# yizhiwang96/Slice3D

Hardware: AMD Instinct MI355X
Metric: occupancy query-points/sec (U-Net encode + per-query decode, 256^2 x 12 slices) (higher is better)
Workload: dtype f16x3

## Files before the change

slice3d_amd/csrc/api.hip:

```cpp
#include <dlfcn.h>
#include <stdarg.h>
#include <string.h>

#include <vector>
#include <mutex>

#include <math.h>

#include "conv_plan.h"
#include "decode.h"
#include "train.h"
#include "ldm_ops.h"

static thread_local char g_err[512] = "";

void s3d_set_error(const char* fmt, ...) {
    va_list ap;
    va_start(ap, fmt);
    vsnprintf(g_err, sizeof(g_err), fmt, ap);
    va_end(ap);
}

extern "C" int s3d_version(void) { return S3D_VERSION; }
extern "C" const char* s3d_last_error(void) { return g_err; }
// ... 85 lines not shown
        tot += ms;
    }
    *total_ms = tot;
    *count = (long)g_prof_ev[id].size();
    return 0;
}

#define TRY(x)              \
    do {                    \
        int rc__ = (x);     \
        if (rc__) return rc__; \
    } while (0)

static const int kEncCin[13] = {3, 64, 64, 128, 128, 256, 256, 256, 512, 512, 512, 512, 512};
static const int kEncCout[13] = {64, 64, 128, 128, 256, 256, 256, 512, 512, 512, 512, 512, 512};
static const bool kEncTap[13] = {false, true, false, true, false, false, true,
                                 false, false, true, false, false, true};
static const int kUpC[4] = {512, 256, 128, 64};

struct PackedConv {
    size_t w, scale, shift;
    size_t w16;
    int cout_pad, KU;
};
struct EncLayout {
    PackedConv enc[13];
    size_t pool_scale[4], pool_shift[4];
};
struct UNetLayout {
    EncLayout E;
    PackedConv trans_up[4], up_t[4], up_c1[4], up_c2[4], outc;
    PackedConv trans_cx, trans_ce;
// ... 182 lines not shown
    }
    TRY(pack_linear(P->outc.w, base + L.outc.w, 3, 16, 32, 32, 0, st));
    TRY(pack_linear(P->outc.w, base + L.outc.w16, 3, 16, 32, 32, 0, st, 1));
    TRY(launch_fold_bn(P->outc.b, nullptr, base + L.outc.scale, base + L.outc.shift, 3, 16, 1, 0, st));
    hipError_t e = hipMemcpyAsync(base + L.emds, P->emds, (size_t)P->n_slices * 128 * sizeof(float),
                                  hipMemcpyDeviceToDevice, st);
    if (e != hipSuccess) {
        s3d_set_error("unet_pack: memcpy failed: %s", hipGetErrorString(e));
        return (int)e;
    }
    return pack_unet_slice_terms(base, L, P->n_slices, st);
}

#define S3D_SPLITK_FLOATS ((size_t)4718592)
struct UNetWs {
    size_t in16, a, b, x[5], p[4], proj, pre, mid, splitk;
    size_t lat, up1_u, up1_pre;
    size_t total;
};
static UNetWs unet_ws(int B, int S, int ns) {
    UNetWs W;
    size_t off = 0;
    auto take = [&](size_t n) {
        size_t o = off;
        off += (n + 63) / 64 * 64;
        return o;
    };
    const size_t px = (size_t)B * S * S;
    W.in16 = take(px * 16);
    W.a = take(px * 64);
    W.b = take(px * 64 / 2);
    const int xc[5] = {64, 128, 256, 512, 512};
    for (int i = 0; i < 5; ++i) W.x[i] = take((px >> (2 * i)) * xc[i]);
    for (int i = 0; i < 4; ++i) W.p[i] = take((px >> (2 * (i + 1))) * xc[i]);
    W.proj = take(px * 32);
    W.pre = take(px * 32);
    W.mid = take(px * ns * 32);
    W.splitk = take(S3D_SPLITK_FLOATS);
    W.lat = take(px / 256 * 512);
    W.up1_u = take(px / 64 * 256);
    W.up1_pre = take(px / 64 * 256);
    W.total = off;
    return W;
}

extern "C" size_t s3d_unet_workspace_bytes(int batch, int size, int n_slices) {
    return unet_ws(batch, size, n_slices).total * sizeof(float);
}

static ConvLaunch conv_desc(const float* base, const PackedConv& pc, int prec, int N, int H, int W, int ks, int act) {
    ConvLaunch c = {};
// ... 38 lines not shown
        c.out_mode = S3D_OUT_CONVT;
        c.cout_store = 256;
        TRY(launch_conv(c, st));
    }
    {
        ConvLaunch c = conv_desc(base, L.up_c1[0], S3D_PREC_F32, ns, 4, 4, 3, S3D_ACT_NONE);
        c.scale = c.shift = nullptr;
        c.nsrc = 1;
        c.src[0] = plain_src(base + L.up1_tab_in, 256);
        c.out = base + L.up1_tab;
        TRY(launch_conv(c, st));
    }
    return 0;
}

static int encoder_fwd(const float* base, const EncLayout& E, int prec, int N, int S, int first, const float* in,
                       float* const tap[5], float* const pp[2], float* const pool[4], float* splitk, hipStream_t st) {
    const float* cur = in;
    int curC = first ? kEncCout[0] : 16, res = S, tap_i = 0, flip = first;
    for (int i = first; i < 13; ++i) {
        ConvLaunch c = conv_desc(base, E.enc[i], prec, N, res, res, 3, kEncTap[i] ? S3D_ACT_NONE : S3D_ACT_RELU);
        c.nsrc = 1;
        c.src[0] = plain_src(cur, curC);
        c.splitk_ws = splitk; c.splitk_floats = S3D_SPLITK_FLOATS;
        c.out = kEncTap[i] ? tap[tap_i] : pp[flip];
        TRY(launch_conv(c, st));
        cur = c.out;
        curC = kEncCout[i];
        if (!kEncTap[i]) {
            flip ^= 1;
            continue;
        }
        if (tap_i < 4) {
            TRY(launch_bn_relu_pool(tap[tap_i], base + E.pool_scale[tap_i], base + E.pool_shift[tap_i], pool[tap_i], N,
                                    res, res, curC, st));
            cur = pool[tap_i];
            res /= 2;
        }
        ++tap_i;
    }
    return 0;
}

extern "C" int s3d_unet_encode_fwd(const void* packed, const float* img, const S3dPyramid* out,
                                   float* slices_rec, int B, int S, int ns, int prec, void* workspace,
                                   size_t workspace_bytes, void* stream) {
    hipStream_t st = (hipStream_t)stream;
    S3D_CHECK_ARG(prec == S3D_PREC_F32 || prec == S3D_PREC_F16X3 || prec == S3D_PREC_F16 || prec == S3D_PREC_BF16,
                  "unet_encode: precision mode %d", prec);
    if (prec == S3D_PREC_BF16) prec = S3D_PREC_F16;
    S3D_CHECK_ARG(packed && img && out && workspace, "unet_encode: null argument");
    S3D_CHECK_ARG(B >= 1 && S >= 16 && S % 16 == 0, "unet_encode: B=%d S=%d (S must be a multiple of 16)", B, S);
    S3D_CHECK_ARG(ns >= 1 && ns <= 12, "unet_encode: n_slices %d", ns);
    S3D_CHECK_ARG(out->n_img == B * ns && out->size == S, "unet_encode: pyramid handle mismatch");
    const UNetLayout L = unet_layout(ns);
    const UNetWs W = unet_ws(B, S, ns);
    if (workspace_bytes < W.total * sizeof(float)) {
        s3d_set_error("unet_encode: workspace %zu < %zu bytes", workspace_bytes, W.total * sizeof(float));
        return S3D_E_WORKSPACE;
    }
    const float* base = (const float*)packed;
    float* ws = (float*)workspace;

    ProfScope prof_(S3D_PROF_UNET, st);
    float* const pp[2] = {ws + W.a, ws + W.b};
    float* const tap[5] = {ws + W.x[0], ws + W.x[1], ws + W.x[2], ws + W.x[3], ws + W.x[4]};
    float* const pool[4] = {ws + W.p[0], ws + W.p[1], ws + W.p[2], ws + W.p[3]};
    TRY(launch_conv3x3_first(img, 3, base + L.enc0_raw, nullptr, pp[0], B, S, S, st, base + L.E.enc[0].scale,
                             base + L.E.enc[0].shift, 1));
    TRY(encoder_fwd(base, L.E, prec, B, S, 1, pp[0], tap, pp, pool, ws + W.splitk, st));
    const int r5 = S / 16;
    {
        ConvLaunch c = conv_desc(base, L.trans_cx, prec, B, r5, r5, 1, S3D_ACT_NONE);
        c.scale = c.shift = nullptr;
        c.nsrc = 1;
        c.src[0] = plain_src(ws + W.x[4], 512);
        c.out = ws + W.lat;
        TRY(launch_conv(c, st));
    }
    TRY(launch_slice_bcast_add(ws + W.lat, base + L.slice_v, out->level[0], B, ns, (long)r5 * r5, 512, st));
    const float* prev = out->level[0];
    int rp = r5;
    for (int i = 0; i < 4; ++i) {
        const int C = kUpC[i], Ct = C / 2, ro = rp * 2;
        {
            ConvLaunch c = conv_desc(base, L.trans_up[i], prec, B, ro, ro, 1, S3D_ACT_NONE);
            c.nsrc = 1;
            c.src[0] = plain_src(ws + W.x[3 - i], C);
            c.out = ws + W.proj;
            TRY(launch_conv(c, st));
        }
        {
            ConvLaunch c = conv_desc(base, L.up_c1s[i], prec, B, ro, ro, 3, S3D_ACT_NONE);
            c.scale = c.shift = nullptr;
            c.nsrc = 1;
            c.src[0] = plain_src(ws + W.proj, Ct);
            c.out = ws + W.pre;
            TRY(launch_conv(c, st));
        }
        if (i == 0) {
            {
                ConvLaunch c = conv_desc(base, L.up_t[0], prec, B, rp, rp, 1, S3D_ACT_NONE);
                c.scale = c.shift = nullptr;
                c.nsrc = 1;
                c.src[0] = plain_src(ws + W.lat, C);
                c.out = ws + W.up1_u;
                c.out_mode = S3D_OUT_CONVT;
                c.cout_store = Ct;
                TRY(launch_conv(c, st));
            }
            {
                ConvLaunch c = conv_desc(base, L.up_c1[0], prec, B, ro, ro, 3, S3D_ACT_NONE);
                c.scale = c.shift = nullptr;
                c.nsrc = 1;
                c.src[0] = plain_src(ws + W.up1_u, Ct);
                c.pre = ws + W.pre; c.pre_bdiv = 1;
                c.out = ws + W.up1_pre;
                TRY(launch_conv(c, st));
            }
            TRY(launch_slice_table_act(ws + W.up1_pre, base + L.up1_tab, base + L.up_c1[0].scale, base + L.up_c1[0].shift,
                                       ws + W.mid, B, ns, ro, Ct, st));
        } else {
            ConvLaunch c = {};
            c.wpk16 = prec != S3D_PREC_F32 ? (const void*)(base + L.up_cc[i].w16) : nullptr;
            c.single_pass = prec == S3D_PREC_F16;
            c.N = B * ns; c.H = rp; c.W = rp; c.ks = 2; c.up2x = 1;
            c.CoutPad = Ct; c.wpk = base + L.up_cc[i].w; c.KU = L.up_cc[i].KU;
            c.scale = base + L.up_c1[i].scale; c.shift = base + L.up_c1[i].shift;
            c.act = S3D_ACT_RELU; c.out_mode = S3D_OUT_NHWC; c.cout_store = Ct; c.out_cstride = Ct;
            c.nsrc = 1;
            c.src[0] = plain_src(prev, C);
            c.pre = ws + W.pre; c.pre_bdiv = ns;
            c.pre_tab = base + L.up_tb[i];
            c.out = ws + W.mid;
            TRY(launch_conv(c, st));
        }
        {
            ConvLaunch c = conv_desc(base, L.up_c2[i], prec, B * ns, ro, ro, 3, S3D_ACT_RELU);
            c.nsrc = 1;
            c.src[0] = plain_src(ws + W.mid, Ct);
            c.out = out->level[i + 1];
            TRY(launch_conv(c, st));
        }
        prev = out->level[i + 1];
        rp = ro;
    }
    if (slices_rec) {
        ConvLaunch c = conv_desc(base, L.outc, prec, B * ns, S, S, 1, S3D_ACT_TANH);
        c.nsrc = 1;
        c.src[0] = plain_src(prev, 32);
        c.out = slices_rec;
        c.out_mode = S3D_OUT_NCHW;
        c.cout_store = 3;
        TRY(launch_conv(c, st));
    }
    return 0;
}

static const int kVggCin[14] = {3, 64, 64, 128, 128, 256, 256, 256, 256, 512, 512, 512, 512, 512};
static const int kVggCout[14] = {64, 64, 128, 128, 256, 256, 256, 256, 512, 512, 512, 512, 512, 512};
static const int kVggPoolAfter[14] = {0, 1, 0, 1, 0, 0, 0, 1, 0, 0, 0, 1, 0, 0};
static const int kVggTap[14] = {0, 1, 0, 2, 0, 3, 0, 0, 0, 4, 0, 0, 0, 5};
static const float kVggW[5] = {1.0f / 2.6f, 1.0f / 4.8f, 1.0f / 3.7f, 1.0f / 5.6f, 10.0f / 1.5f};

struct VggLayout {
    PackedConv conv[14];
    size_t mean, stdv, total;
};
static VggLayout vgg_layout() {
    VggLayout L;
    size_t off = 0;
// ... 279 lines not shown
    return false;
}

extern "C" size_t s3d_decode_workspace_bytes(int batch, long n_qry, int n_slices) {
    return decode_ws(batch, n_qry, n_slices, S3D_CHUNK_GROUPS).total * sizeof(float);
}
extern "C" size_t s3d_decode_workspace_bytes_min(int batch, long n_qry, int n_slices) {
    return decode_ws(batch, n_qry, n_slices, S3D_CHUNK_GROUPS_MIN).total * sizeof(float);
}

struct DecodeLanes {
    std::mutex mu;
    hipStream_t aux = nullptr;
    hipEvent_t stagger = nullptr, join = nullptr;
    bool ok = false;
};
static std::atomic<int> g_decode_lanes{-1};
extern "C" int s3d_decode_set_lanes(int n) {
    S3D_CHECK_ARG(n == 1 || n == 2, "decode_set_lanes: %d (1 or 2)", n);
    g_decode_lanes.store(n, std::memory_order_relaxed);
    return 0;
}
static int decode_lanes() {
    int v = g_decode_lanes.load(std::memory_order_relaxed);
    if (v < 0) {
        const char* e = getenv("S3D_DECODE_LANES");
        v = (e && atoi(e) == 2) ? 2 : 1;
        g_decode_lanes.store(v, std::memory_order_relaxed);
    }
    return v;
// ... 8 lines not shown
    if (L.ok) return true;
    hipStream_t s = nullptr;
    hipEvent_t e0 = nullptr, e1 = nullptr;
    const bool made = hipStreamCreateWithFlags(&s, hipStreamNonBlocking) == hipSuccess &&
                      hipEventCreateWithFlags(&e0, hipEventDisableTiming) == hipSuccess &&
                      hipEventCreateWithFlags(&e1, hipEventDisableTiming) == hipSuccess;
    if (!made) {
        if (e1) (void)hipEventDestroy(e1);
        if (e0) (void)hipEventDestroy(e0);
        if (s) (void)hipStreamDestroy(s);
        (void)hipGetLastError();
        return false;
    }
    L.aux = s; L.stagger = e0; L.join = e1; L.ok = true;
    return true;
}
#define S3D_LANES_MIN_GROUPS 8192

static LayerPtrs layer_ptrs(const float* b, const HeadLayout& H, int l) {
    LayerPtrs p;
    p.inw = b + H.L[l].inw; p.inb = b + H.L[l].inb; p.outw = b + H.L[l].outw; p.outb = b + H.L[l].outb;
    p.ln1g = b + H.L[l].ln1g; p.ln1b = b + H.L[l].ln1b; p.w1 = b + H.L[l].w1; p.b1 = b + H.L[l].b1;
    p.w2 = b + H.L[l].w2; p.b2 = b + H.L[l].b2; p.ln2g = b + H.L[l].ln2g; p.ln2b = b + H.L[l].ln2b;
    p.wf16 = b + H.L[l].wf16;
    p.aq16 = b + H.L[l].aq16;
    p.wfb16 = b + H.L[l].wfb16;
    p.aqb16 = b + H.L[l].aqb16;
    return p;
}

// ... 309 lines not shown

extern "C" int s3d_nchw_to_nhwc(const float* in, float* out, int n, int c, int h, int w, void* stream) {
    S3D_CHECK_ARG(in && out, "nchw_to_nhwc: null argument");
    return launch_nchw_to_nhwc(in, out, n, c, h, w, c, (hipStream_t)stream);
}

extern "C" int s3d_nhwc_to_nchw(const float* in, float* out, int n, int c, int h, int w, void* stream) {
    S3D_CHECK_ARG(in && out, "nhwc_to_nchw: null argument");
    return launch_nhwc_to_nchw(in, out, n, c, h, w, (hipStream_t)stream);
}

#include "api_gt.inc"
#include "api_ldm.inc"
#include "api_ldm_ae.inc"
#include "api_train.inc"
#include "api_train_gt.inc"
```

slice3d_amd/csrc/conv.h:

```cpp
#pragma once
#include "common.h"
#include "dropout.h"

struct ConvSrc {
    const float* p;
    int C;
    int bdiv, bmod, sbcast;
};

#define S3D_GN_SLICES 64
#define S3D_GN_CMAX 1536
struct ConvGn {
    const float* table;
    int silu;
};

enum { S3D_ACT_NONE = 0, S3D_ACT_RELU = 1, S3D_ACT_TANH = 2 };
enum { S3D_OUT_NHWC = 0, S3D_OUT_CONVT = 1, S3D_OUT_NCHW = 2 };

struct ConvLaunch {
    ConvSrc src[2];
    int nsrc;
    int N, H, W;
    int ks;
// ... 17 lines not shown
    int xcd_remap;
    const float* gate;
    float gate_scale;
    unsigned long long drop_base;
    float* splitk_ws;
    size_t splitk_floats;
    DropCfg drop;
    ConvGn gn;
    const float* pre;
    int pre_bdiv, pre_bmod;
    int* splits_out;
    int up2x;
    const float* pre_tab;
    int tap_oy, tap_ox;
    int out_py, out_px;
};

int launch_conv(const ConvLaunch& a, hipStream_t stream);
int launch_conv_splitk_finish(const ConvLaunch& a, int nsplit, hipStream_t stream);

enum { S3D_PACK_LINEAR = 0, S3D_PACK_CONV = 1, S3D_PACK_CONVT = 2, S3D_PACK_CONV_DGRAD = 3,
       S3D_PACK_CONVT_DGRAD = 4, S3D_PACK_LINEAR_T = 5 };
struct PackArgs {
    const float* src;
    float* dst;
    int kind;
    int n_valid, n_pad;
    int KU_total, u_off, ku_seg;
    int ld, k_valid;
    int taps, cseg, cseg_valid, cin_tot, cin_begin;
// ... 45 lines not shown
```

slice3d_amd/csrc/conv.hip:

```cpp
#include <stdlib.h>
#include "conv_plan.h"
#include <utility>
#include <vector>

template <int MT, int NT>
__device__ __forceinline__ void conv_epilogue(const ConvLaunch& a, f32x4 (&acc)[MT][NT], const int (&pn)[MT],
                                              const int (&py)[MT], const int (&px)[MT], const bool (&pv)[MT],
                                              int jt0, int g) {
    const bool convt32 = a.out_mode == S3D_OUT_CONVT && a.cout_store % 32 == 0;
    if (NT % 2 == 0 && (a.out_mode == S3D_OUT_NHWC || convt32)) {
        const int m = threadIdx.x & 15;
        const bool lo = m < 8;
#pragma unroll
        for (int np = 0; np < NT / 2; ++np) {
            const int co = (jt0 + 2 * np) * 16 + 16 * (m >> 3) + 4 * g;
            const f32x4 sc = a.scale ? ld4(a.scale + co) : f32x4{1.f, 1.f, 1.f, 1.f};
            const f32x4 sh = a.shift ? ld4(a.shift + co) : zero4();
            const int ct = a.cout_store, cq = convt32 ? co / ct : 0, ccol = convt32 ? co - cq * ct : co;
            const bool col_ok = convt32 ? cq < 4 : co < a.cout_store;
#pragma unroll
            for (int mt = 0; mt < MT; ++mt) {
                f32x4 val[2];
                s3d_full_line_pair(acc[mt][2 * np], acc[mt][2 * np + 1], m, val[0], val[1]);
                const long ob = convt32 ? ((long)(pn[mt] * 2 * a.H + 2 * py[mt] + (cq >> 1)) * (2 * a.W) + 2 * px[mt] + (cq & 1)) * ct
// ... 1067 lines not shown
            const f32x4 v0 = ld4(src + (size_t)k * stride), v1 = ld4(src + (size_t)(k + 1) * stride),
                        v2 = ld4(src + (size_t)(k + 2) * stride), v3 = ld4(src + (size_t)(k + 3) * stride);
            __builtin_amdgcn_sched_barrier(0);
            s += (v0 + v1) + (v2 + v3);
        }
        for (; k < nsplit; ++k) s += ld4(src + (size_t)k * stride);
        f32x4 acc[1][1] = {{s}};
        const int n = (int)(p / ((long)a.H * a.W));
        const int r = (int)(p - (long)n * a.H * a.W);
        const int pn[1] = {n}, py[1] = {r / a.W}, px[1] = {r % a.W};
        const bool pv[1] = {true};
        conv_epilogue<1, 1>(a, acc, pn, py, px, pv, co >> 4, (co >> 2) & 3);
    }
}

int launch_conv_splitk_finish(const ConvLaunch& a, int nsplit, hipStream_t stream) {
    hipLaunchKernelGGL(conv_splitk_finish_kernel, dim3(conv_splitk_finish_blocks(a)), dim3(256), 0, stream, a, nsplit);
    S3D_LAUNCH_CHECK();
    return 0;
}


#define C3S_HP 160
#define C3S_HP1 64
__device__ __forceinline__ int c3s_div(int q, int magic) { return (q * magic) >> 16; }
template <int PT, bool GN, int TAPS = 9>
__global__ __launch_bounds__(256) void conv3x3_small_f16x3_kernel(const ConvLaunch a, int chunks_per_split) {
    constexpr int BORD = TAPS == 9 ? 1 : 0;
    __shared__ __attribute__((aligned(16))) _Float16 s_in[2][2][C3S_HP * C3_PXS];
    const int lane = threadIdx.x & 63, wave = threadIdx.x >> 6;
    const int m = lane & 15, g = lane >> 4;
// ... 194 lines not shown
        if (e.family == p.family && std::equal(e.targ, e.targ + 7, p.targ)) {
            k = &e;
            break;
        }
    S3D_CHECK_ARG(k, "conv: the plan names a kernel instantiation that is not built");
    for (int par = 0; par < (p.per_parity ? 4 : 1); ++par) {
        if (p.per_parity) {
            a.wpk = a_in.wpk + (size_t)par * (a.CoutPad / 16) * a.KU * 256;
            a.out_py = par >> 1; a.out_px = par & 1;
            a.tap_oy = a.out_py - 1; a.tap_ox = a.out_px - 1;
        }
        k->launch(a, p, stream);
        S3D_LAUNCH_CHECK();
    }
    if (a.splits_out) *a.splits_out = p.splits;
    return p.finish ? launch_conv_splitk_finish(a, p.splits, stream) : 0;
}
#undef CK_ARGS
#undef CK
#undef CK_TILE
#undef CK_LDS
#undef CK_SMALL
#undef CK_UP2X
#undef CK_STREAM

__device__ __forceinline__ void pack_frag_body(const PackArgs& a) {
    const long total = (long)(a.n_pad / 16) * a.ku_seg * 256;
    for (long idx = (long)blockIdx.x * blockDim.x + threadIdx.x; idx < total;
         idx += (long)gridDim.x * blockDim.x) {
        int e, lane, ul, j, k;
        if (!a.f16) {
// ... 490 lines not shown
```

slice3d_amd/csrc/conv_plan.h:

```cpp
#pragma once
#include <stdlib.h>
#include <algorithm>
#include "conv.h"

struct ConvTuning {
    bool small3_on, small1_on;
    long small3_pmax, small1_pmax;
};
inline ConvTuning conv_tuning_from_env() {
    const char *e3 = getenv("S3D_CONV_SMALL"), *e1 = getenv("S3D_CONV_SMALL_1X1");
    const int v3 = e3 ? atoi(e3) : 1, v1 = e1 ? atoi(e1) : 1;
    return {v3 != 0, v1 != 0, v3 > 1 ? v3 : 32, v1 > 1 ? v1 : 64};
}
const ConvTuning& conv_tuning();

enum ConvFamily { CONV_IGEMM, CONV_IGEMM_F16X3, CONV_LIN_ROWS, CONV_LIN_STREAM, CONV_LDS, CONV_SMALL, CONV_UP2X_LDS, CONV_N_FAMILIES };
static const struct { const char* name; int nargs; const char* bools; } kConvFamily[CONV_N_FAMILIES] = {
    {"conv_igemm_kernel", 7, "0000011"},       {"conv_igemm_f16x3_kernel", 6, "000001"}, {"lin_rows_f16x3_kernel", 0, ""},
    {"lin_stream_f16x3_kernel", 1, "0"},       {"conv3x3_lds_f16x3_kernel", 6, "000011"}, {"conv3x3_small_f16x3_kernel", 3, "010"},
    {"conv_up2x_lds_f16x3_kernel", 7, "0000000"}};

struct ConvPlan {
    int err;
    ConvFamily family;
    int targ[7];
    unsigned grid_x, grid_y, block;
    int splits, chunks_per_split;
    int tiles_x, tiles_y;
    long n_tasks;
    bool finish;
    bool per_parity;
};

constexpr long kSmallHalo = 160, kSmallHalo1 = 64;
constexpr int kLinRowsTile = 192;

inline bool conv_same_grid(const ConvLaunch& a) { return !((a.Hin && a.Hin != a.H) || (a.Win && a.Win != a.W)); }
inline bool conv_chunked_sources(const ConvLaunch& a) {
    for (int s = 0; s < a.nsrc; ++s)
        if (a.src[s].C % 32 || a.src[s].sbcast) return false;
    return true;
}
inline bool conv_splittable(const ConvLaunch& a) { return a.splitk_ws && a.out_mode == S3D_OUT_NHWC; }
inline bool conv_below_lds_tile(int H, int W) { return W < 16 || H < 8; }
inline int conv_splitk_finish_blocks(const ConvLaunch& a) {
    const long total = (long)(((size_t)a.N * a.H * a.W * a.CoutPad) >> 2);
    return (int)((total + 255) / 256 < 2048 ? (total + 255) / 256 : 2048);
}

inline void conv_plan_splits(ConvPlan& p, const ConvLaunch& a, long nblk_k, bool may_split) {
    int nchunk = 0;
    for (int s = 0; s < a.nsrc; ++s) nchunk += a.src[s].C >> 5;
    const size_t out_floats = (size_t)a.N * a.H * a.W * a.CoutPad;
    int splits = 1;
    long best = -1;
    for (int sp = 1; may_split && sp <= nchunk && (size_t)sp * out_floats <= a.splitk_floats; ++sp) {
        const int c = (nchunk + sp - 1) / sp, se = (nchunk + c - 1) / c;
        if (se != sp) continue;
        const long rounds = (nblk_k * se + 511) / 512;
        const long cost = rounds * (2 * c + 3) + (se > 1 ? 1 + se / 8 : 0);
        if (best < 0 || cost < best) {
// ... 17 lines not shown

inline int conv_plan_route(const ConvLaunch& a, const ConvTuning& t, ConvPlan& p) {
    S3D_CHECK_ARG(a.ks >= 1 && a.ks <= 3, "conv: ks must be 1, 2 or 3");
    S3D_CHECK_ARG(!a.pad_origin || (a.ks == 3 && a.stride > 1 && a.out_mode == S3D_OUT_NHWC),
                  "conv: pad_origin is served for strided 3x3 convolutions only");
    S3D_CHECK_ARG(a.CoutPad % 16 == 0 && a.CoutPad > 0, "conv: CoutPad %d", a.CoutPad);
    for (int s = 0; s < a.nsrc; ++s)
        S3D_CHECK_ARG(a.src[s].C % 16 == 0 && a.src[s].bdiv >= 1, "conv: bad source %d", s);
    S3D_CHECK_ARG(a.out_mode != S3D_OUT_CONVT || (a.drop.p <= 0.f && !a.gate && !a.residual && !a.out_accumulate),
                  "conv: ConvTranspose output takes no dropout / gate / residual / accumulate");
    S3D_CHECK_ARG(!a.pre || a.up2x || (a.ks == 3 && a.stride <= 1 && !a.Hin && !a.Win), "conv: a pre-activation addend is served for 3x3 stride-1 convolutions only");
    S3D_CHECK_ARG(!a.pre || a.out_mode != S3D_OUT_CONVT, "conv: a pre-activation addend with a ConvTranspose output");
    S3D_CHECK_ARG(!a.pre || !a.splitk_ws, "conv: a pre-activation addend with a split-K workspace");
    S3D_CHECK_ARG(!a.pre || !a.gn.table, "conv: a pre-activation addend with a fused GroupNorm");
    S3D_CHECK_ARG(!a.pre || (a.pre_bdiv >= 1 && a.pre_bmod >= 0), "conv: addend image rule bdiv %d bmod %d", a.pre_bdiv, a.pre_bmod);
    const long P = (long)a.N * a.H * a.W;
    p.tiles_x = (a.W + 15) / 16; p.tiles_y = (a.H + 7) / 8;
    const long tiles = (long)p.tiles_x * p.tiles_y * a.N;
    const int co_wg = a.CoutPad % 64 == 0 ? 64 : 32;

    if (a.up2x) {
        S3D_CHECK_ARG(a.ks == 2 && a.stride <= 1 && !a.Hin && !a.Win, "conv: the composed ConvTranspose -> 3x3 is a 2x2 stride-1 form (ks %d)", a.ks);
        S3D_CHECK_ARG(!a.splitk_ws && !a.splits_out, "conv: the composed ConvTranspose -> 3x3 with a split-K workspace");
        S3D_CHECK_ARG(!a.gn.table, "conv: the composed ConvTranspose -> 3x3 with a fused GroupNorm");
        S3D_CHECK_ARG(a.out_mode == S3D_OUT_NHWC && a.cout_store == a.CoutPad, "conv: the composed ConvTranspose -> 3x3 stores NHWC, all channels");
        S3D_CHECK_ARG(a.pre && a.pre_tab, "conv: the composed ConvTranspose -> 3x3 needs its addend and its border-class table");
        S3D_CHECK_ARG(a.nsrc == 1 && !a.src[0].sbcast && a.src[0].C % 32 == 0 && a.CoutPad % 32 == 0 && a.KU == a.src[0].C / 4,
                      "conv: the composed ConvTranspose -> 3x3 takes one plain source (C %d, Cout %d, KU %d)", a.src[0].C, a.CoutPad, a.KU);
        S3D_CHECK_ARG(!a.pad_origin && a.out_cstride >= a.CoutPad && a.src[0].bdiv >= 1 && a.src[0].bmod >= 0 && a.pre_bdiv >= 1 && a.pre_bmod >= 0,
                      "conv: the composed ConvTranspose -> 3x3: pad_origin %d, channel stride %d < %d, or a bad image rule", a.pad_origin, a.out_cstride, a.CoutPad);
// ... 75 lines not shown
        const long nblk = ((P + pix - 1) / pix) * (a.CoutPad / co);
        if (a.CoutPad % m.mod || nblk < m.want) continue;
        CONV_GRID_CHECK(nblk, 1);
        conv_plan_kernel(p, f16 ? CONV_IGEMM_F16X3 : CONV_IGEMM, {m.MT, m.NT, m.WM, m.WN, a.ks, a.pre != nullptr, 0}, nblk, 1, m.WM * m.WN * 64);
        return 0;
    }
    return 0;
}
#undef CONV_GRID_CHECK

inline ConvPlan conv_plan(const ConvLaunch& a, const ConvTuning& t) {
    ConvPlan p = {};
    p.splits = 1;
    p.err = conv_plan_route(a, t, p);
    p.finish = p.splits > 1 && !a.splits_out;
    return p;
}

inline void conv_plan_describe(const ConvLaunch& a, const ConvPlan& p, char* buf, size_t len) {
    const auto& f = kConvFamily[p.family];
    size_t n = (size_t)snprintf(buf, len, "%s%s", f.name, f.nargs ? "<" : "");
    for (int i = 0; i < f.nargs && n < len; ++i) {
        const char* sep = i + 1 < f.nargs ? "," : ">";
        if (f.bools[i] == '1') n += (size_t)snprintf(buf + n, len - n, "%s%s", p.targ[i] ? "true" : "false", sep);
        else n += (size_t)snprintf(buf + n, len - n, "%d%s", p.targ[i], sep);
    }
    if (n < len) n += (size_t)snprintf(buf + n, len - n, " grid=%ux%u block=%u splits=%d finish=%d%s", p.grid_x, p.grid_y, p.block, p.splits, (int)p.finish, p.per_parity ? " launches=4" : "");
    if (p.finish && n < len) snprintf(buf + n, len - n, "; conv_splitk_finish_kernel grid=%dx1 block=256", conv_splitk_finish_blocks(a));
}
```

Before: 11.73 million.

## Run U-Net skip branches on a side stream and fuse pooling into encoder convs

```diff
diff --git a/slice3d_amd/csrc/api.hip b/slice3d_amd/csrc/api.hip
--- a/slice3d_amd/csrc/api.hip
+++ b/slice3d_amd/csrc/api.hip
@@ -4,6 +4,7 @@
 
 #include <vector>
 #include <mutex>
+#include <string>
 
 #include <math.h>
 
@@ -123,8 +124,6 @@
 
 static const int kEncCin[13] = {3, 64, 64, 128, 128, 256, 256, 256, 512, 512, 512, 512, 512};
 static const int kEncCout[13] = {64, 64, 128, 128, 256, 256, 256, 512, 512, 512, 512, 512, 512};
-static const bool kEncTap[13] = {false, true, false, true, false, false, true,
-                                 false, false, true, false, false, true};
 static const int kUpC[4] = {512, 256, 128, 64};
 
 struct PackedConv {
@@ -337,7 +336,7 @@
 
 #define S3D_SPLITK_FLOATS ((size_t)4718592)
 struct UNetWs {
-    size_t in16, a, b, x[5], p[4], proj, pre, mid, splitk;
+    size_t in16, a, b, x[5], p[4], proj, pre[4], mid, splitk;
     size_t lat, up1_u, up1_pre;
     size_t total;
 };
@@ -357,7 +356,7 @@
     for (int i = 0; i < 5; ++i) W.x[i] = take((px >> (2 * i)) * xc[i]);
     for (int i = 0; i < 4; ++i) W.p[i] = take((px >> (2 * (i + 1))) * xc[i]);
     W.proj = take(px * 32);
-    W.pre = take(px * 32);
+    for (int i = 0; i < 4; ++i) W.pre[i] = take((px >> (2 * (3 - i))) * (256 >> i));
     W.mid = take(px * ns * 32);
     W.splitk = take(S3D_SPLITK_FLOATS);
     W.lat = take(px / 256 * 512);
@@ -426,37 +425,53 @@
     return 0;
 }
 
+static int launch_or_describe(const ConvLaunch& c, hipStream_t st, std::string* dry) {
+    if (!dry) return launch_conv(c, st);
+    const ConvPlan p = conv_plan(c, conv_tuning());
+    if (p.err) return p.err;
+    char text[512];
+    conv_plan_describe(c, p, text, sizeof(text));
+    *dry += text;
+    return 0;
+}
+static int enc_conv_step(const float* base, const EncLayout& E, int prec, int N, int S, const UNetStep& s, float* const buf[UB_N],
+                         hipStream_t st, std::string* dry = nullptr) {
+    const int i = s.idx, res = S >> s.down;
+    ConvLaunch c = conv_desc(base, E.enc[i], prec, N, res, res, 3, kEncTap[i] ? S3D_ACT_NONE : S3D_ACT_RELU);
+    c.nsrc = 1;
+    c.src[0] = plain_src(buf[s.rd[0]], i ? kEncCin[i] : 16);
+    c.splitk_ws = buf[UB_SPLITK]; c.splitk_floats = S3D_SPLITK_FLOATS;
+    c.out = buf[s.wr[0]];
+    if (s.wr[1] >= 0) {
+        const int t = s.wr[1] - UB_P1;
+        c.pool_out = buf[s.wr[1]]; c.pool_scale = base + E.pool_scale[t]; c.pool_shift = base + E.pool_shift[t];
+    }
+    return launch_or_describe(c, st, dry);
+}
+
 static int encoder_fwd(const float* base, const EncLayout& E, int prec, int N, int S, int first, const float* in,
                        float* const tap[5], float* const pp[2], float* const pool[4], float* splitk, hipStream_t st) {
-    const float* cur = in;
-    int curC = first ? kEncCout[0] : 16, res = S, tap_i = 0, flip = first;
-    for (int i = first; i < 13; ++i) {
-        ConvLaunch c = conv_desc(base, E.enc[i], prec, N, res, res, 3, kEncTap[i] ? S3D_ACT_NONE : S3D_ACT_RELU);
-        c.nsrc = 1;
-        c.src[0] = plain_src(cur, curC);
-        c.splitk_ws = splitk; c.splitk_floats = S3D_SPLITK_FLOATS;
-        c.out = kEncTap[i] ? tap[tap_i] : pp[flip];
-        TRY(launch_conv(c, st));
-        cur = c.out;
-        curC = kEncCout[i];
-        if (!kEncTap[i]) {
-            flip ^= 1;
-            continue;
-        }
-        if (tap_i < 4) {
-            TRY(launch_bn_relu_pool(tap[tap_i], base + E.pool_scale[tap_i], base + E.pool_shift[tap_i], pool[tap_i], N,
-                                    res, res, curC, st));
-            cur = pool[tap_i];
-            res /= 2;
-        }
-        ++tap_i;
-    }
-    return 0;
-}
-
-extern "C" int s3d_unet_encode_fwd(const void* packed, const float* img, const S3dPyramid* out,
-                                   float* slices_rec, int B, int S, int ns, int prec, void* workspace,
-                                   size_t workspace_bytes, void* stream) {
+    float* buf[UB_N] = {};
+    buf[first ? UB_A : UB_IN16] = const_cast<float*>(in);
+    if (!first) buf[UB_A] = pp[0];
+    buf[UB_B] = pp[1];
+    for (int k = 0; k < 5; ++k) buf[UB_X1 + k] = tap[k];
+    for (int k = 0; k < 4; ++k) buf[UB_P1 + k] = pool[k];
+    buf[UB_SPLITK] = splitk;
+    std::vector<UNetStep> steps;
+    unet_enc_steps(first, steps);
+    for (const UNetStep& s : steps) TRY(enc_conv_step(base, E, prec, N, S, s, buf, st));
+    return 0;
+}
+
+struct UNetSide {
+    hipStream_t aux = nullptr;
+    hipEvent_t fork = nullptr, join[kUNetMarks] = {};
+};
+static int unet_side_acquire(std::unique_lock<std::mutex>& lock, UNetSide& side);
+
+static int unet_encode_impl(const void* packed, const float* img, const S3dPyramid* out, float* slices_rec, int B, int S, int ns,
+                            int prec, void* workspace, size_t workspace_bytes, void* stream, bool serial, std::string* dry = nullptr) {
     hipStream_t st = (hipStream_t)stream;
     S3D_CHECK_ARG(prec == S3D_PREC_F32 || prec == S3D_PREC_F16X3 || prec == S3D_PREC_F16 || prec == S3D_PREC_BF16,
                   "unet_encode: precision mode %d", prec);
@@ -473,66 +488,117 @@
     }
     const float* base = (const float*)packed;
     float* ws = (float*)workspace;
+    float* buf[UB_N] = {};
+    buf[UB_IMG] = const_cast<float*>(img);
+    buf[UB_A] = ws + W.a; buf[UB_B] = ws + W.b;
+    for (int k = 0; k < 5; ++k) buf[UB_X1 + k] = ws + W.x[k], buf[UB_LV0 + k] = (float*)out->level[k];
+    for (int k = 0; k < 4; ++k) buf[UB_P1 + k] = ws + W.p[k], buf[UB_PRE1 + k] = ws + W.pre[k];
+    buf[UB_SPLITK] = ws + W.splitk; buf[UB_LAT] = ws + W.lat; buf[UB_PROJ] = ws + W.proj;
+    buf[UB_UP1_U] = ws + W.up1_u; buf[UB_UP1_PRE] = ws + W.up1_pre; buf[UB_MID] = ws + W.mid; buf[UB_REC] = slices_rec;
 
     ProfScope prof_(S3D_PROF_UNET, st);
-    float* const pp[2] = {ws + W.a, ws + W.b};
-    float* const tap[5] = {ws + W.x[0], ws + W.x[1], ws + W.x[2], ws + W.x[3], ws + W.x[4]};
-    float* const pool[4] = {ws + W.p[0], ws + W.p[1], ws + W.p[2], ws + W.p[3]};
-    TRY(launch_conv3x3_first(img, 3, base + L.enc0_raw, nullptr, pp[0], B, S, S, st, base + L.E.enc[0].scale,
-                             base + L.E.enc[0].shift, 1));
-    TRY(encoder_fwd(base, L.E, prec, B, S, 1, pp[0], tap, pp, pool, ws + W.splitk, st));
-    const int r5 = S / 16;
-    {
-        ConvLaunch c = conv_desc(base, L.trans_cx, prec, B, r5, r5, 1, S3D_ACT_NONE);
-        c.scale = c.shift = nullptr;
-        c.nsrc = 1;
-        c.src[0] = plain_src(ws + W.x[4], 512);
-        c.out = ws + W.lat;
-        TRY(launch_conv(c, st));
-    }
-    TRY(launch_slice_bcast_add(ws + W.lat, base + L.slice_v, out->level[0], B, ns, (long)r5 * r5, 512, st));
-    const float* prev = out->level[0];
-    int rp = r5;
-    for (int i = 0; i < 4; ++i) {
-        const int C = kUpC[i], Ct = C / 2, ro = rp * 2;
-        {
+    const std::vector<UNetStep> steps = unet_encode_schedule(!serial, slices_rec != nullptr);
+    std::unique_lock<std::mutex> side_lock;
+    UNetSide side;
+    bool forked = false;
+    int rc = 0, last_mark = -1;
+    auto hip_rc = [](const char* what, hipError_t e) {
+        if (e != hipSuccess) s3d_set_error("%s: %s", what, hipGetErrorString(e));
+        return (int)e;
+    };
+    for (const UNetStep& s : steps)
+        if (s.op == UO_MARK) last_mark = s.idx;
+    for (const UNetStep& s : steps) {
+        hipStream_t q = s.side ? side.aux : st;
+        if (dry) {
+            char line[160];
+            unet_schedule_describe({s}, line, sizeof(line));
+            dry->append(line, strlen(line) - 1);
+            *dry += " | ";
+        }
+        const int i = s.idx, r5 = S / 16, rp = r5 << (i & 3), ro = rp * 2, C = kUpC[i & 3], Ct = C / 2;
+        const float* in0 = s.rd[0] >= 0 ? buf[s.rd[0]] : nullptr;
+        float* o = s.wr[0] >= 0 ? buf[s.wr[0]] : nullptr;
+        switch (s.op) {
+        case UO_FORK:
+            rc = dry ? 0 : unet_side_acquire(side_lock, side);
+            if (!rc && !dry) {
+                S3D_HIP_TRY("unet_encode: fork", hipEventRecord(side.fork, st));
+                S3D_HIP_TRY("unet_encode: fork", hipStreamWaitEvent(side.aux, side.fork, 0));
+                forked = true;
+            }
+            break;
+        case UO_MARK:
+            if (!dry) rc = hip_rc("unet_encode: mark", hipEventRecord(side.join[s.idx], side.aux));
+            break;
+        case UO_JOIN:
+            if (dry) break;
+            rc = hip_rc("unet_encode: join", hipStreamWaitEvent(st, side.join[s.idx], 0));
+            if (!rc && s.idx == last_mark) {
+                forked = false;
+                side_lock.unlock();
+            }
+            break;
+        case UO_ENC_FIRST:
+            if (!dry) rc = launch_conv3x3_first(img, 3, base + L.enc0_raw, nullptr, o, B, S, S, q, base + L.E.enc[0].scale, base + L.E.enc[0].shift, 1);
+            break;
+        case UO_ENC_CONV:
+            rc = enc_conv_step(base, L.E, prec, B, S, s, buf, q, dry);
+            break;
+        case UO_TRANS_C: {
+            ConvLaunch c = conv_desc(base, L.trans_cx, prec, B, r5, r5, 1, S3D_ACT_NONE);
+            c.scale = c.shift = nullptr;
+            c.nsrc = 1;
+            c.src[0] = plain_src(in0, 512);
+            c.out = o;
+            rc = launch_or_describe(c, q, dry);
+            break;
+        }
+        case UO_BCAST:
+            if (!dry) rc = launch_slice_bcast_add(in0, base + L.slice_v, o, B, ns, (long)r5 * r5, 512, q);
+            break;
+        case UO_SKIP_PROJ: {
             ConvLaunch c = conv_desc(base, L.trans_up[i], prec, B, ro, ro, 1, S3D_ACT_NONE);
             c.nsrc = 1;
-            c.src[0] = plain_src(ws + W.x[3 - i], C);
-            c.out = ws + W.proj;
-            TRY(launch_conv(c, st));
-        }
-        {
+            c.src[0] = plain_src(in0, C);
+            c.out = o;
+            rc = launch_or_describe(c, q, dry);
+            break;
+        }
+        case UO_SKIP_3X3: {
             ConvLaunch c = conv_desc(base, L.up_c1s[i], prec, B, ro, ro, 3, S3D_ACT_NONE);
             c.scale = c.shift = nullptr;
             c.nsrc = 1;
-            c.src[0] = plain_src(ws + W.proj, Ct);
-            c.out = ws + W.pre;
-            TRY(launch_conv(c, st));
-        }
-        if (i == 0) {
-            {
-                ConvLaunch c = conv_desc(base, L.up_t[0], prec, B, rp, rp, 1, S3D_ACT_NONE);
-                c.scale = c.shift = nullptr;
-                c.nsrc = 1;
-                c.src[0] = plain_src(ws + W.lat, C);
-                c.out = ws + W.up1_u;
-                c.out_mode = S3D_OUT_CONVT;
-                c.cout_store = Ct;
-                TRY(launch_conv(c, st));
-            }
-            {
-                ConvLaunch c = conv_desc(base, L.up_c1[0], prec, B, ro, ro, 3, S3D_ACT_NONE);
-                c.scale = c.shift = nullptr;
-                c.nsrc = 1;
-                c.src[0] = plain_src(ws + W.up1_u, Ct);
-                c.pre = ws + W.pre; c.pre_bdiv = 1;
-                c.out = ws + W.up1_pre;
-                TRY(launch_conv(c, st));
-            }
-            TRY(launch_slice_table_act(ws + W.up1_pre, base + L.up1_tab, base + L.up_c1[0].scale, base + L.up_c1[0].shift,
-                                       ws + W.mid, B, ns, ro, Ct, st));
-        } else {
+            c.src[0] = plain_src(in0, Ct);
+            c.out = o;
+            rc = launch_or_describe(c, q, dry);
+            break;
+        }
+        case UO_UP1_CONVT: {
+            ConvLaunch c = conv_desc(base, L.up_t[0], prec, B, rp, rp, 1, S3D_ACT_NONE);
+            c.scale = c.shift = nullptr;
+            c.nsrc = 1;
+            c.src[0] = plain_src(in0, C);
+            c.out = o;
+            c.out_mode = S3D_OUT_CONVT;
+            c.cout_store = Ct;
+            rc = launch_or_describe(c, q, dry);
+            break;
+        }
+        case UO_UP1_3X3: {
+            ConvLaunch c = conv_desc(base, L.up_c1[0], prec, B, ro, ro, 3, S3D_ACT_NONE);
+            c.scale = c.shift = nullptr;
+            c.nsrc = 1;
+            c.src[0] = plain_src(in0, Ct);
+            c.pre = buf[s.rd[1]]; c.pre_bdiv = 1;
+            c.out = o;
+            rc = launch_or_describe(c, q, dry);
+            break;
+        }
+        case UO_UP1_TABLE:
+            if (!dry) rc = launch_slice_table_act(in0, base + L.up1_tab, base + L.up_c1[0].scale, base + L.up_c1[0].shift, o, B, ns, ro, Ct, q);
+            break;
+        case UO_UP2X: {
             ConvLaunch c = {};
             c.wpk16 = prec != S3D_PREC_F32 ? (const void*)(base + L.up_cc[i].w16) : nullptr;
             c.single_pass = prec == S3D_PREC_F16;
@@ -541,32 +607,48 @@
             c.scale = base + L.up_c1[i].scale; c.shift = base + L.up_c1[i].shift;
             c.act = S3D_ACT_RELU; c.out_mode = S3D_OUT_NHWC; c.cout_store = Ct; c.out_cstride = Ct;
             c.nsrc = 1;
-            c.src[0] = plain_src(prev, C);
-            c.pre = ws + W.pre; c.pre_bdiv = ns;
+            c.src[0] = plain_src(in0, C);
+            c.pre = buf[s.rd[1]]; c.pre_bdiv = ns;
             c.pre_tab = base + L.up_tb[i];
-            c.out = ws + W.mid;
-            TRY(launch_conv(c, st));
-        }
-        {
+            c.out = o;
+            rc = launch_or_describe(c, q, dry);
+            break;
+        }
+        case UO_UP_C2: {
             ConvLaunch c = conv_desc(base, L.up_c2[i], prec, B * ns, ro, ro, 3, S3D_ACT_RELU);
             c.nsrc = 1;
-            c.src[0] = plain_src(ws + W.mid, Ct);
-            c.out = out->level[i + 1];
-            TRY(launch_conv(c, st));
-        }
-        prev = out->level[i + 1];
-        rp = ro;
-    }
-    if (slices_rec) {
-        ConvLaunch c = conv_desc(base, L.outc, prec, B * ns, S, S, 1, S3D_ACT_TANH);
-        c.nsrc = 1;
-        c.src[0] = plain_src(prev, 32);
-        c.out = slices_rec;
-        c.out_mode = S3D_OUT_NCHW;
-        c.cout_store = 3;
-        TRY(launch_conv(c, st));
-    }
-    return 0;
+            c.src[0] = plain_src(in0, Ct);
+            c.out = o;
+            rc = launch_or_describe(c, q, dry);
+            break;
+        }
+        case UO_OUTC: {
+            ConvLaunch c = conv_desc(base, L.outc, prec, B * ns, S, S, 1, S3D_ACT_TANH);
+            c.nsrc = 1;
+            c.src[0] = plain_src(in0, 32);
+            c.out = o;
+            c.out_mode = S3D_OUT_NCHW;
+            c.cout_store = 3;
+            rc = launch_or_describe(c, q, dry);
+            break;
+        }
+        default:
+            S3D_CHECK_ARG(false, "unet_encode: schedule step %d", s.op);
+        }
+        if (dry) *dry += "\n";
+        if (rc) break;
+    }
+    if (forked) {
+        S3D_HIP_TRY("unet_encode: join", hipEventRecord(side.join[0], side.aux));
+        S3D_HIP_TRY("unet_encode: join", hipStreamWaitEvent(st, side.join[0], 0));
+    }
+    return rc;
+}
+
+extern "C" int s3d_unet_encode_fwd(const void* packed, const float* img, const S3dPyramid* out,
+                                   float* slices_rec, int B, int S, int ns, int prec, void* workspace,
+                                   size_t workspace_bytes, void* stream) {
+    return unet_encode_impl(packed, img, out, slices_rec, B, S, ns, prec, workspace, workspace_bytes, stream, false);
 }
 
 static const int kVggCin[14] = {3, 64, 64, 128, 128, 256, 256, 256, 256, 512, 512, 512, 512, 512};
@@ -876,6 +958,8 @@
     hipStream_t aux = nullptr;
     hipEvent_t stagger = nullptr, join = nullptr;
     bool ok = false;
+    UNetSide unet;
+    bool unet_ok = false;
 };
 static std::atomic<int> g_decode_lanes{-1};
 extern "C" int s3d_decode_set_lanes(int n) {
@@ -914,6 +998,31 @@
     }
     L.aux = s; L.stagger = e0; L.join = e1; L.ok = true;
     return true;
+}
+static int unet_side_acquire(std::unique_lock<std::mutex>& lock, UNetSide& side) {
+    DecodeLanes* L = decode_lanes_for_device();
+    S3D_CHECK_ARG(L, "unet_encode: hipGetDevice failed");
+    lock = std::unique_lock<std::mutex>(L->mu);
+    if (!L->unet_ok) {
+        UNetSide u;
+        hipError_t e = hipStreamCreateWithFlags(&u.aux, hipStreamNonBlocking);
+        if (e == hipSuccess) e = hipEventCreateWithFlags(&u.fork, hipEventDisableTiming);
+        for (hipEvent_t& j : u.join)
+            if (e == hipSuccess) e = hipEventCreateWithFlags(&j, hipEventDisableTiming);
+        if (e != hipSuccess) {
+            for (hipEvent_t j : u.join)
+                if (j) (void)hipEventDestroy(j);
+            if (u.fork) (void)hipEventDestroy(u.fork);
+            if (u.aux) (void)hipStreamDestroy(u.aux);
+            (void)hipGetLastError();
+            lock.unlock();
+            S3D_HIP_TRY("unet_encode: side stream", e);
+        }
+        L->unet = u;
+        L->unet_ok = true;
+    }
+    side = L->unet;
+    return 0;
 }
 #define S3D_LANES_MIN_GROUPS 8192
 
@@ -1253,4 +1362,7 @@
 #include "api_ldm.inc"
 #include "api_ldm_ae.inc"
 #include "api_train.inc"
+#ifdef S3D_TEST_EXPORTS
+#include "api_test.inc"
+#endif
 #include "api_train_gt.inc"
diff --git a/slice3d_amd/csrc/conv.h b/slice3d_amd/csrc/conv.h
--- a/slice3d_amd/csrc/conv.h
+++ b/slice3d_amd/csrc/conv.h
@@ -55,6 +55,8 @@
     const float* pre_tab;
     int tap_oy, tap_ox;
     int out_py, out_px;
+    float* pool_out;
+    const float* pool_scale, *pool_shift;
 };
 
 int launch_conv(const ConvLaunch& a, hipStream_t stream);
diff --git a/slice3d_amd/csrc/conv.hip b/slice3d_amd/csrc/conv.hip
--- a/slice3d_amd/csrc/conv.hip
+++ b/slice3d_amd/csrc/conv.hip
@@ -1105,7 +1105,62 @@
     }
 }
 
+__global__ void conv_splitk_finish_pool_kernel(const ConvLaunch a, int nsplit) {
+    const long P = (long)a.N * a.H * a.W;
+    const int cq = a.CoutPad >> 2, ho = a.H >> 1, wo = a.W >> 1;
+    const long total = (long)a.N * ho * wo * cq;
+    const size_t stride = (size_t)P * a.CoutPad;
+    for (long idx = (long)blockIdx.x * blockDim.x + threadIdx.x; idx < total; idx += (long)gridDim.x * blockDim.x) {
+        const int co = (int)(idx % cq) * 4;
+        long r = idx / cq;
+        const int x = (int)(r % wo);
+        r /= wo;
+        const int y = (int)(r % ho);
+        const int n = (int)(r / ho);
+        const f32x4 sc = a.scale ? ld4(a.scale + co) : f32x4{1.f, 1.f, 1.f, 1.f};
+        const f32x4 sh = a.shift ? ld4(a.shift + co) : zero4();
+        const f32x4 psc = a.pool_scale ? ld4(a.pool_scale + co) : f32x4{1.f, 1.f, 1.f, 1.f};
+        const f32x4 psh = a.pool_shift ? ld4(a.pool_shift + co) : zero4();
+        f32x4 best;
+#pragma unroll
+        for (int t = 0; t < 4; ++t) {
+            const long p = ((long)n * a.H + 2 * y + (t >> 1)) * a.W + 2 * x + (t & 1);
+            const float* src = a.splitk_ws + (size_t)p * a.CoutPad + co;
+            f32x4 s = zero4();
+            int k = 0;
+            for (; k + 4 <= nsplit; k += 4) {
+                const f32x4 v0 = ld4(src + (size_t)k * stride), v1 = ld4(src + (size_t)(k + 1) * stride),
+                            v2 = ld4(src + (size_t)(k + 2) * stride), v3 = ld4(src + (size_t)(k + 3) * stride);
+                __builtin_amdgcn_sched_barrier(0);
+                s += (v0 + v1) + (v2 + v3);
+            }
+            for (; k < nsplit; ++k) s += ld4(src + (size_t)k * stride);
+            f32x4 v = s * sc + sh;
+            if (a.act == S3D_ACT_RELU) {
+#pragma unroll
+                for (int i = 0; i < 4; ++i) v[i] = fmaxf(v[i], 0.f);
+            }
+            __builtin_nontemporal_store(v, reinterpret_cast<f32x4*>(a.out + p * a.CoutPad + co));
+            f32x4 u = v * psc + psh;
+#pragma unroll
+            for (int i = 0; i < 4; ++i) {
+                u[i] = fmaxf(u[i], 0.f);
+                best[i] = t == 0 ? u[i] : fmaxf(best[i], u[i]);
+            }
+        }
+        st4(a.pool_out + idx * 4, best);
+    }
+}
+
 int launch_conv_splitk_finish(const ConvLaunch& a, int nsplit, hipStream_t stream) {
+    if (a.pool_out) {
+        S3D_CHECK_ARG(a.out_mode == S3D_OUT_NHWC && a.cout_store == a.CoutPad && a.out_cstride == a.CoutPad && a.H % 2 == 0 && a.W % 2 == 0 &&
+                          a.CoutPad % 4 == 0 && a.drop.p <= 0.f && !a.gate && !a.residual && !a.out_accumulate && a.act != S3D_ACT_TANH,
+                      "conv finish: a pooled output takes a plain NHWC output of all channels on an even map, scale / shift / ReLU only");
+        hipLaunchKernelGGL(conv_splitk_finish_pool_kernel, dim3(conv_splitk_finish_pool_blocks(a)), dim3(256), 0, stream, a, nsplit);
+        S3D_LAUNCH_CHECK();
+        return 0;
+    }
     hipLaunchKernelGGL(conv_splitk_finish_kernel, dim3(conv_splitk_finish_blocks(a)), dim3(256), 0, stream, a, nsplit);
     S3D_LAUNCH_CHECK();
     return 0;
@@ -1330,7 +1385,8 @@
         S3D_LAUNCH_CHECK();
     }
     if (a.splits_out) *a.splits_out = p.splits;
-    return p.finish ? launch_conv_splitk_finish(a, p.splits, stream) : 0;
+    if (p.finish) return launch_conv_splitk_finish(a, p.splits, stream);
+    return p.pool_after ? launch_bn_relu_pool(a.out, a.pool_scale, a.pool_shift, a.pool_out, a.N, a.H, a.W, a.CoutPad, stream) : 0;
 }
 #undef CK_ARGS
 #undef CK
diff --git a/slice3d_amd/csrc/conv_plan.h b/slice3d_amd/csrc/conv_plan.h
--- a/slice3d_amd/csrc/conv_plan.h
+++ b/slice3d_amd/csrc/conv_plan.h
@@ -1,6 +1,7 @@
 #pragma once
 #include <stdlib.h>
 #include <algorithm>
+#include <vector>
 #include "conv.h"
 
 struct ConvTuning {
@@ -29,6 +30,8 @@
     int tiles_x, tiles_y;
     long n_tasks;
     bool finish;
+    bool finish_pool;
+    bool pool_after;
     bool per_parity;
 };
 
@@ -45,6 +48,10 @@
 inline bool conv_below_lds_tile(int H, int W) { return W < 16 || H < 8; }
 inline int conv_splitk_finish_blocks(const ConvLaunch& a) {
     const long total = (long)(((size_t)a.N * a.H * a.W * a.CoutPad) >> 2);
+    return (int)((total + 255) / 256 < 2048 ? (total + 255) / 256 : 2048);
+}
+inline int conv_splitk_finish_pool_blocks(const ConvLaunch& a) {
+    const long total = (long)(((size_t)a.N * a.H * a.W * a.CoutPad) >> 4);
     return (int)((total + 255) / 256 < 2048 ? (total + 255) / 256 : 2048);
 }
 
@@ -92,6 +99,9 @@
     S3D_CHECK_ARG(!a.pre || !a.splitk_ws, "conv: a pre-activation addend with a split-K workspace");
     S3D_CHECK_ARG(!a.pre || !a.gn.table, "conv: a pre-activation addend with a fused GroupNorm");
     S3D_CHECK_ARG(!a.pre || (a.pre_bdiv >= 1 && a.pre_bmod >= 0), "conv: addend image rule bdiv %d bmod %d", a.pre_bdiv, a.pre_bmod);
+    S3D_CHECK_ARG(!a.pool_out || (a.out_mode == S3D_OUT_NHWC && a.cout_store == a.CoutPad && a.out_cstride == a.CoutPad && a.H % 2 == 0 && a.W % 2 == 0 &&
+                                  !a.up2x && !a.splits_out && a.drop.p <= 0.f && !a.gate && !a.residual && !a.out_accumulate && a.act != S3D_ACT_TANH),
+                  "conv: a pooled output takes a plain NHWC output of all channels on an even map, scale / shift / ReLU only");
     const long P = (long)a.N * a.H * a.W;
     p.tiles_x = (a.W + 15) / 16; p.tiles_y = (a.H + 7) / 8;
     const long tiles = (long)p.tiles_x * p.tiles_y * a.N;
@@ -197,6 +207,8 @@
     p.splits = 1;
     p.err = conv_plan_route(a, t, p);
     p.finish = p.splits > 1 && !a.splits_out;
+    p.finish_pool = p.finish && a.pool_out;
+    p.pool_after = !p.err && a.pool_out && !p.finish;
     return p;
 }
 
@@ -209,5 +221,143 @@
         else n += (size_t)snprintf(buf + n, len - n, "%d%s", p.targ[i], sep);
     }
     if (n < len) n += (size_t)snprintf(buf + n, len - n, " grid=%ux%u block=%u splits=%d finish=%d%s", p.grid_x, p.grid_y, p.block, p.splits, (int)p.finish, p.per_parity ? " launches=4" : "");
-    if (p.finish && n < len) snprintf(buf + n, len - n, "; conv_splitk_finish_kernel grid=%dx1 block=256", conv_splitk_finish_blocks(a));
-}
+    if (p.finish_pool && n < len) n += (size_t)snprintf(buf + n, len - n, "; conv_splitk_finish_pool_kernel grid=%dx1 block=256", conv_splitk_finish_pool_blocks(a));
+    else if (p.finish && n < len) n += (size_t)snprintf(buf + n, len - n, "; conv_splitk_finish_kernel grid=%dx1 block=256", conv_splitk_finish_blocks(a));
+    if (p.pool_after && n < len) snprintf(buf + n, len - n, "; bn_relu_pool_kernel");
+}
+
+enum UNetBuf { UB_IMG, UB_IN16, UB_A, UB_B, UB_X1, UB_X2, UB_X3, UB_X4, UB_X5, UB_P1, UB_P2, UB_P3, UB_P4, UB_SPLITK, UB_LAT,
+               UB_LV0, UB_LV1, UB_LV2, UB_LV3, UB_LV4, UB_PROJ, UB_PRE1, UB_PRE2, UB_PRE3, UB_PRE4, UB_UP1_U, UB_UP1_PRE, UB_MID,
+               UB_REC, UB_N };
+static const char* const kUNetBufName[UB_N] = {"img", "in16", "a", "b", "x1", "x2", "x3", "x4", "x5", "p1", "p2", "p3", "p4", "splitk", "lat",
+                                               "lv0", "lv1", "lv2", "lv3", "lv4", "proj", "pre1", "pre2", "pre3", "pre4", "up1_u", "up1_pre",
+                                               "mid", "rec"};
+enum UNetOp { UO_ENC_FIRST, UO_ENC_CONV, UO_TRANS_C, UO_BCAST, UO_SKIP_PROJ, UO_SKIP_3X3, UO_UP1_CONVT, UO_UP1_3X3, UO_UP1_TABLE,
+              UO_UP2X, UO_UP_C2, UO_OUTC, UO_FORK, UO_MARK, UO_JOIN, UO_N };
+constexpr int kUNetMarks = 4;
+static const char* const kUNetOpName[UO_N] = {"enc_first", "enc_conv", "trans_c", "slice_bcast_add", "skip_proj", "skip_3x3", "up1_convt",
+                                              "up1_3x3", "slice_table_act", "up2x", "up_c2", "outc", "fork", "mark", "join"};
+struct UNetStep {
+    int op, idx;
+    int side;
+    int rd[2], wr[3];
+    int down;
+};
+constexpr bool kEncTap[13] = {false, true, false, true, false, false, true, false, false, true, false, false, true};
+
+inline void unet_enc_steps(int first, std::vector<UNetStep>& out) {
+    int cur = first ? UB_A : UB_IN16, down = 0, tap_i = 0, flip = first;
+    for (int i = first; i < 13; ++i) {
+        UNetStep s = {UO_ENC_CONV, i, 0, {cur, -1}, {kEncTap[i] ? UB_X1 + tap_i : (flip ? UB_B : UB_A), -1, UB_SPLITK}, down};
+        cur = s.wr[0];
+        if (!kEncTap[i]) flip ^= 1;
+        else {
+            if (tap_i < 4) {
+                cur = s.wr[1] = UB_P1 + tap_i;
+                ++down;
+            }
+            ++tap_i;
+        }
+        out.push_back(s);
+    }
+}
+inline unsigned unet_step_reads(const UNetStep& s) {
+    unsigned m = 0;
+    for (int b : s.rd) m |= b >= 0 ? 1u << b : 0u;
+    return m;
+}
+inline unsigned unet_step_writes(const UNetStep& s) {
+    unsigned m = 0;
+    for (int b : s.wr) m |= b >= 0 ? 1u << b : 0u;
+    return m;
+}
+inline bool unet_step_in_branch(const UNetStep& s) { return s.op == UO_SKIP_PROJ || s.op == UO_SKIP_3X3; }
+
+inline std::vector<UNetStep> unet_encode_serial(bool want_rec) {
+    std::vector<UNetStep> v;
+    v.push_back({UO_ENC_FIRST, 0, 0, {UB_IMG, -1}, {UB_A, -1, -1}, 0});
+    unet_enc_steps(1, v);
+    v.push_back({UO_TRANS_C, 0, 0, {UB_X5, -1}, {UB_LAT, -1, -1}, 0});
+    v.push_back({UO_BCAST, 0, 0, {UB_LAT, -1}, {UB_LV0, -1, -1}, 0});
+    for (int i = 0; i < 4; ++i) {
+        v.push_back({UO_SKIP_PROJ, i, 0, {UB_X4 - i, -1}, {UB_PROJ, -1, -1}, 0});
+        v.push_back({UO_SKIP_3X3, i, 0, {UB_PROJ, -1}, {UB_PRE1 + i, -1, -1}, 0});
+        if (i == 0) {
+            v.push_back({UO_UP1_CONVT, 0, 0, {UB_LAT, -1}, {UB_UP1_U, -1, -1}, 0});
+            v.push_back({UO_UP1_3X3, 0, 0, {UB_UP1_U, UB_PRE1}, {UB_UP1_PRE, -1, -1}, 0});
+            v.push_back({UO_UP1_TABLE, 0, 0, {UB_UP1_PRE, -1}, {UB_MID, -1, -1}, 0});
+        } else {
+            v.push_back({UO_UP2X, i, 0, {UB_LV0 + i, UB_PRE1 + i}, {UB_MID, -1, -1}, 0});
+        }
+        v.push_back({UO_UP_C2, i, 0, {UB_MID, -1}, {UB_LV1 + i, -1, -1}, 0});
+    }
+    if (want_rec) v.push_back({UO_OUTC, 0, 0, {UB_LV4, -1}, {UB_REC, -1, -1}, 0});
+    return v;
+}
+
+inline std::vector<UNetStep> unet_encode_schedule(bool fork, bool want_rec) {
+    const std::vector<UNetStep> serial = unet_encode_serial(want_rec);
+    if (!fork) return serial;
+    unsigned br_rd = 0, br_wr = 0;
+    for (const UNetStep& s : serial)
+        if (unet_step_in_branch(s)) br_rd |= unet_step_reads(s), br_wr |= unet_step_writes(s);
+    const unsigned ext_in = br_rd & ~br_wr;
+    const int n = (int)serial.size();
+    int fork_at = 0, first_branch = n;
+    unsigned read_outside = 0;
+    for (int j = 0; j < n; ++j) {
+        const UNetStep& s = serial[j];
+        if (unet_step_in_branch(s)) {
+            first_branch = std::min(first_branch, j);
+            continue;
+        }
+        if (unet_step_writes(s) & ext_in) fork_at = j + 1;
+        read_outside |= unet_step_reads(s) & br_wr;
+    }
+    if (fork_at > first_branch || !read_outside) return serial;
+    std::vector<UNetStep> v(serial.begin(), serial.begin() + fork_at);
+    v.push_back({UO_FORK, 0, 0, {-1, -1}, {-1, -1, -1}, 0});
+    int n_marks = 0, mark_of[UB_N] = {};
+    for (UNetStep s : serial)
+        if (unet_step_in_branch(s)) {
+            s.side = 1;
+            v.push_back(s);
+            if (!(unet_step_writes(s) & read_outside)) continue;
+            if (n_marks == kUNetMarks) return serial;
+            for (int b : s.wr)
+                if (b >= 0) mark_of[b] = n_marks;
+            v.push_back({UO_MARK, n_marks++, 1, {-1, -1}, {-1, -1, -1}, 0});
+        }
+    int joined = -1;
+    for (int j = fork_at; j < n; ++j) {
+        const UNetStep& s = serial[j];
+        if (unet_step_in_branch(s)) continue;
+        if (unet_step_writes(s) & (br_rd | br_wr)) return serial;
+        int need = -1;
+        for (int b : s.rd)
+            if (b >= 0 && (br_wr >> b & 1u)) {
+                if (!(read_outside >> b & 1u)) return serial;
+                need = std::max(need, mark_of[b]);
+            }
+        if (need > joined) v.push_back({UO_JOIN, joined = need, 0, {-1, -1}, {-1, -1, -1}, 0});
+        v.push_back(s);
+    }
+    if (joined != n_marks - 1) return serial;
+    return v;
+}
+
+inline void unet_schedule_describe(const std::vector<UNetStep>& steps, char* buf, size_t len) {
+    size_t n = 0;
+    if (len) buf[0] = 0;
+    for (const UNetStep& s : steps) {
+        if (n < len) n += (size_t)snprintf(buf + n, len - n, "%s %s[%d] r=", s.side ? "side" : "main", kUNetOpName[s.op], s.idx);
+        const char* sep = "";
+        for (int b : s.rd)
+            if (b >= 0 && n < len) n += (size_t)snprintf(buf + n, len - n, "%s%s", sep, kUNetBufName[b]), sep = ",";
+        if (n < len) n += (size_t)snprintf(buf + n, len - n, " w=");
+        sep = "";
+        for (int b : s.wr)
+            if (b >= 0 && n < len) n += (size_t)snprintf(buf + n, len - n, "%s%s", sep, kUNetBufName[b]), sep = ",";
+        if (n < len) n += (size_t)snprintf(buf + n, len - n, "\n");
+    }
+}
```

New measurement: 11.70 million. Within noise of the previous version (-0.3%).
